# Henweiz/MARL-Responsible-Nav

Hardware: AMD Instinct MI355X
Metric: agent-env-steps/sec at 64k envs × 4 agents, 1/2/4/8 MI355X; HBM BW fraction (higher is better)
Workload: dtype int32

## Files before the change

### include/gridenv.h

```cpp
#ifndef GRIDENV_H
#define GRIDENV_H
#include <stdint.h>

#ifdef __cplusplus
extern "C" {
#endif

#define GW_MAX_AGENTS 8
#define GW_N_ACTIONS 9

typedef enum gw_status {
    GW_OK = 0,
    GW_ERR_ARG = -1,
    GW_ERR_HIP = -2,
    GW_ERR_ALLOC = -3,
    GW_ERR_STATE = -4
} gw_status;

typedef struct gw_scenario {
    int32_t H, W;
    const uint8_t *region;
    const uint8_t *policy_id;
    int32_t n_policies;
    const double *policy_cdf;
// ... 33 lines not shown
    int32_t *mdr;
    int32_t *final_pos;
    uint8_t *crash_bits;
    uint8_t *restr_bits;
    double *stats;
    uint8_t *done_copy;
    double *stats_acc;
    int64_t *tick;
    uint32_t *desc_copy;
    double *fear_row;
} gw_step_out;

#define GW_STATS 8

typedef struct gw_state {
    int32_t *pos;
    uint32_t *flags;
    int32_t *t;
    uint32_t *episode;
    int32_t *prev_dist;
    double *score;
    double *fear_score;
} gw_state;

gw_status gw_create(const gw_scenario *sc, const gw_config *cfg, int device, void **out_env);

gw_status gw_reset(void *env, const uint8_t *env_mask, const int32_t *spawn_cells, float *obs,
                   uint16_t *mask, void *stream);

gw_status gw_step(void *env, const int32_t *rl_actions, const int32_t *scripted,
                  const int32_t *spawn, const gw_step_out *out, void *stream);

gw_status gw_state_view(void *env, gw_state *out);

gw_status gw_copy_state(void *env, const gw_state *buf, int to_env, void *stream);

enum {
    GW_SPAN_STEP = 0, GW_SPAN_OBS = 1, GW_SPAN_FEAR = 2, GW_SPAN_ACT = 3, GW_SPAN_CNN_L1 = 4,
    GW_SPAN_CNN_LIST = 5, GW_SPAN_CNN_RARE = 6, GW_SPAN_WINDOW = 7, GW_SPAN_LEARN = 8,
    GW_SPAN_FEAR_ALT = 9, GW_SPAN_FEAL = 10, GW_SPAN_FEAR_FULL = 11, GW_SPAN_FEAR_PREVIEW = 12
};
gw_status gw_profile(void *env, int enable);
gw_status gw_profile_read(void *env, double out_ms[3], int64_t *n_steps);
gw_status gw_profile_spans(void *env, double *out, int64_t cap, int64_t *n_spans);

gw_status gw_fear_matrix(void *env, int64_t n, const int32_t *cells, const int32_t *actions,
                         const int32_t *mdr, const uint8_t *in_list, double *resp, int32_t *vm,
                         int32_t *va, double *feal, int32_t *feal_vm, int32_t *feal_va, void *stream);

int64_t gw_stats_rows(void *env);

int64_t gw_kernel_path(void *env);

gw_status gw_graph_replayed(void *env, void *stream);

int64_t gw_pipeline_state_bytes(void);
gw_status gw_pipeline_save(void *env, void *buf);
gw_status gw_pipeline_load(void *env, const void *buf, void *stream);

typedef struct gw_obs_source {
    const uint32_t *desc;
    const float *base;
    int32_t apples[GW_MAX_AGENTS];
    int32_t N, K, H, W, variant;
    int64_t E, env_offset;
} gw_obs_source;
gw_status gw_obs_view(void *env, gw_obs_source *out);

gw_status gw_obs_desc_copy(void *env, uint32_t *dst, void *stream);

gw_status gw_count_sims(void *env, uint64_t *counter);

gw_status gw_set_fear_alt(void *env, double *fear_alt);

gw_status gw_set_feal(void *env, double *feal, uint16_t *feal_valid);

gw_status gw_set_fear_full(void *env, double *resp_full, uint16_t *resp_valid);

gw_status gw_fear_preview(void *env, const int32_t *rl_actions, const int32_t *scripted, double *fear_alt,
                          int32_t *actions, int32_t *mdr, void *stream);

gw_status gw_obs_patch(void *env, int32_t P, float *patch, float *final_patch, void *stream);
gw_status gw_step_patch_next(void *env, int32_t P, float *patch, float *final_patch);

gw_status gw_set_obs_async(void *env, int enable);

enum { GW_OBS_F32 = 0, GW_OBS_BF16 = 1 };
gw_status gw_set_obs_dtype(void *env, int dtype);

#define GW_OBS_DESTS 8
gw_status gw_set_obs_delta(void *env, int on);
gw_status gw_obs_dest_forget(void *env, const void *ptr);
gw_status gw_obs_delta_counts(void *env, int64_t out[2]);

gw_status gw_set_fear_blocks(void *env, int wide);
gw_status gw_obs_fence(void *env, void *stream);
gw_status gw_fear_fence(void *env, void *stream);
void gw_set_last_error(const char *msg);
gw_status gw_dims(void *env, int64_t out[5]);

const char *gw_last_error(void);

void gw_destroy(void *env);

#ifdef __cplusplus
}
// ... 3 lines not shown
```

### marl-responsible-nav_amd/csrc/gridenv.hip

```cpp
#include <hip/hip_runtime.h>
#include <hip/hip_ext.h>

#include <cstdint>
#include <cstdio>
#include <cstdlib>
#include <algorithm>
#include <cstring>
#include <new>
#include <type_traits>
#include <string>
#include <vector>

#include "patch_ops.h"
#include "gridenv.h"
#include "prof.h"
#include "dispatch.h"
#include "obs_value.h"
#include "obs_dest.h"
#include "philox.h"
#include "window_rows.h"
#include "fear_alt_tasks.h"
#include "resp_tables.h"
#include "cf_env.h"

// ... 693 lines not shown
        nf = nw[1].x;
        ocells = ds[0];
        of = saved[e * NDESC + 4];
    }
    __syncthreads();
    if (!live || !(nf & D_WRITE)) return;
    if (k == 0) {
        uint4 *ds = reinterpret_cast<uint4 *>(saved + e * NDESC);
        ds[0] = nw[0];
        ds[1] = nw[1];
        ds[2] = nw[2];
    }
    PatchSet nu, od;
    decode_patches(p, nw[0], nf, k, nu);
    decode_patches(p, ocells, of, k, od);
    float *o = obs + ((int64_t)k * p.E + e) * HW;
#pragma unroll
    for (int q = 0; q < NPATCH_MAX; ++q) {
        const int c = nu.c[q];
        bool st = (unsigned)c < (unsigned)HW;
#pragma unroll
        for (int q2 = q + 1; q2 < NPATCH_MAX; ++q2) st = st && nu.c[q2] != c;
        bool held = false;
        float ov = 0.0f;
#pragma unroll
        for (int q2 = 0; q2 < NPATCH_MAX; ++q2) {
            const bool m = od.c[q2] == c;
            held = held || m;
            ov = m ? od.v[q2] : ov;
        }
        if (st && !(held && ov == nu.v[q])) o[c] = nu.v[q];
    }
#pragma unroll
    for (int q = 0; q < NPATCH_MAX; ++q) {
        const int c = od.c[q];
        bool st = (unsigned)c < (unsigned)HW;
#pragma unroll
        for (int q2 = 0; q2 < q; ++q2) st = st && od.c[q2] != c;
#pragma unroll
        for (int q2 = 0; q2 < NPATCH_MAX; ++q2) st = st && nu.c[q2] != c;
        if (st) o[c] = ((p.tb.roadbits[c >> 5] >> (c & 31)) & 1u) ? 0.0f : -1.0f;
    }
}

#ifndef GW_NOFEAR_BE
#define GW_NOFEAR_BE 32
#endif
#ifndef GW_DEF_BE
#define GW_DEF_BE 128
#endif
#ifndef GW_FEAR_T
#define GW_FEAR_T 256
#endif
template <int N, int KMAX, bool FEAR, bool WIDE = false, bool DEF = false, int TT = 128> struct V2Cfg {
    static constexpr int THREADS = TT;
    static constexpr int BE = (WIDE ? 2 : 1) *
        (FEAR ? (KMAX <= 2 ? (N <= 4 ? 32 : 16) : (N <= 4 ? 16 : 4))
              : (KMAX <= 2 && N > 4 ? 128 : (DEF && KMAX <= 2 ? GW_DEF_BE : GW_NOFEAR_BE)));
    static constexpr bool XDRAW = !FEAR && BE <= 32 && N <= 4;
    static_assert(!FEAR || BE * KMAX <= THREADS, "fear_block: one lane per (env, actor)");
    static_assert(!FEAR || BE <= 64, "task encoding holds 6 env bits");
    static constexpr int MAXB = FEAR ? BE * (1 + 2 * KMAX) : 1;
    static constexpr int MAXG = FEAR ? BE * KMAX * (N > 1 ? N - 1 : 1) : 1;
    using Task = typename std::conditional<(KMAX <= 2), uint16_t, uint32_t>::type;
    static __device__ __forceinline__ Task enc(int el, int k, int j, int var, int b) {
        return (Task)((uint32_t)el | ((uint32_t)b << 6) | ((uint32_t)var << 10) | ((uint32_t)j << 11) |
                      ((uint32_t)k << 14));
    }
};

template <int N, int KMAX, bool FEAR, bool WIDE = false, bool DEF = false, int TT = 128>
struct alignas(16) V2Shared {
    using Cfg = V2Cfg<N, KMAX, FEAR, WIDE, DEF, TT>;
    static constexpr int BE = Cfg::BE, FB = FEAR ? BE : 1;
    double red[Cfg::THREADS / 64][GW_STATS];
    typename Cfg::Task tasks[Cfg::MAXB];
    typename Cfg::Task groups[Cfg::MAXG];
    int pos[FB][N];
    int fin[FB][N];
    int apple[FB][KMAX];
    uint32_t bits[FB];
    int8_t act[FB][N];
    int8_t mdr[FB][N];
    uint8_t close[FB][KMAX];
    uint32_t vset[FB][KMAX][FEAR ? N : 1];
    uint2 wl[(N >= GW_LIST_MIN_N) ? Cfg::THREADS * N : 1];
    int8_t xact[Cfg::XDRAW ? BE : 1][N];
    int8_t xmdr[Cfg::XDRAW ? BE : 1][N];
    int nbase, ngroup;
};

#include "draw_action.h"

template <int N>
__device__ __forceinline__ void select_actions_v2(const Params &p, int64_t e, const EnvState<N> &es,
                                                  const uint32_t *ctab, const double *cdf_s, int (&act)[N]) {
#pragma unroll
    for (int n = 0; n < N; ++n) act[n] = draw_action(p, e, n, es.episode, es.t, es.pos[n], ctab, cdf_s);
}

template <int N, int KMAX, class Sh>
__device__ __forceinline__ void fear_plan_actor(const Params &p, Sh &sh, int el, int k, const int (&pos)[N],
                                                const int (&act)[N], int mdr_k, int off0) {
    using Cfg = typename Sh::Cfg;
    int pk = pos[0], ak = act[0];
#pragma unroll
    for (int n = 1; n < N; ++n) {
        pk = (n == k) ? pos[n] : pk;
        ak = (n == k) ? act[n] : ak;
    }
    uint32_t close = 0;
#pragma unroll
    for (int n = 0; n < N; ++n)
        if (n == k || manhattan(p, pk, pos[n]) <= 5) close |= 1u << n;
    sh.close[el][k] = (uint8_t)close;
#pragma unroll
    for (int n = 0; n < N; ++n) sh.vset[el][k][n] = 0u;
    if (ak == mdr_k) return;
    const int ng = __popc(close) - 1;
    int sb = off0 + atomicAdd(&sh.nbase, 2);
    int sg = ng ? atomicAdd(&sh.ngroup, ng) : 0;
    sh.tasks[sb] = Cfg::enc(el, k, 0, 0, 15);
    sh.tasks[sb + 1] = Cfg::enc(el, k, 0, 1, 15);
#pragma unroll
    for (int j = 0; j < N; ++j)
        if (j != k && ((close >> j) & 1u)) sh.groups[sg++] = Cfg::enc(el, k, j, 0, 0);
}

template <class Sh>
__device__ __forceinline__ uint32_t fear_task_at(const Sh &sh, int ti, int nb_end) {
    if (ti < nb_end) return sh.tasks[ti];
    const int g = (ti - nb_end) >> 4, s = (ti - nb_end) & 15;
    const uint32_t tk = sh.groups[g];
    const int el = tk & 63, j = (tk >> 11) & 7;
    const int bi = s & 7;
    const int b = bi + (bi >= (int)sh.act[el][j]);
    return tk | ((uint32_t)b << 6) | ((uint32_t)(s >> 3) << 10);
}

template <int N, class Sh>
__device__ __forceinline__ void fear_record(Sh &sh, int el, int k, int j, int var, int b, uint32_t valid) {
    const int sft = 16 * var;
    if (b != 15) {
        if ((valid >> j) & 1u) atomicOr(&sh.vset[el][k][j], 1u << (sft + b));
        return;
    }
    const uint32_t cl = sh.close[el][k];
#pragma unroll
    for (int n = 0; n < N; ++n) {
        if (n == k || !((valid >> n) & 1u)) continue;
        const uint32_t bits = ((cl >> n) & 1u) ? 1u << (int)sh.act[el][n] : 0x1FFu;
        atomicOr(&sh.vset[el][k][n], bits << sft);
    }
}

template <int N, int KMAX, class Sh, class OK>
__device__ __forceinline__ void fear_task(const Params &p, Sh &sh, uint32_t tk, const OK &okv) {
    const int el = tk & 63, b = (tk >> 6) & 15, var = (tk >> 10) & 1, j = (tk >> 11) & 7, k = (int)(tk >> 14);
    int pos[N], joint[N], fin[N];
    const uint32_t cl = sh.close[el][k];
#pragma unroll
    for (int n = 0; n < N; ++n) {
        pos[n] = sh.pos[el][n];
        joint[n] = ((cl >> n) & 1u) ? (int)sh.act[el][n] : 0;
        if (n == k && var == 0) joint[n] = sh.mdr[el][n];
        if (n == j && b != 15) joint[n] = b;
    }
    int apple[MAXN];
#pragma unroll
    for (int q = 0; q < MAXN; ++q) apple[q] = -1;
    constexpr bool LIST = N >= GW_LIST_MIN_N;
    World<N, LIST> w;
    w.init(pos, joint, p.W, p.w_magic);
    if constexpr (LIST) w.lw = &sh.wl[threadIdx.x * N];
    uint32_t caught;
    simulate<N, true>(w, okv, 0, apple, caught, fin);
    fear_record<N>(sh, el, k, j, var, b, ~(w.crash | w.restr) & ((1u << N) - 1u));
}

template <int N, int KMAX, class Sh>
__device__ __forceinline__ double fear_value(const Params &p, const Sh &sh, int el, int64_t e, int k, bool skipped,
                                             const double *resp_s) {
    double *row = p.out.fear_row ? p.out.fear_row + (e * p.K + k) * N : nullptr;
    if (skipped) {
        if (row)
#pragma unroll
            for (int jj = 0; jj < N; ++jj) row[jj] = 0.0;
        return 0.0;
    }
    double resp[N];
#pragma unroll
    for (int jj = 0; jj < N; ++jj) {
        resp[jj] = 0.0;
        if (jj != k) {
            const uint32_t v = sh.vset[el][k][jj];
            resp[jj] = resp_s[__popc(v & 0x1FFu) * 10 + __popc(v >> 16)];
        }
        if (row) row[jj] = resp[jj];
    }
    double sum = 0.0;
#pragma unroll
    for (int kk = 0; kk < KMAX; ++kk)
        if (kk == k) sum = np_sum_row<N>(resp, kk);
    return sum;
}

template <int T, uint32_t FM = 0xFFu, uint32_t IM = 0u>
__device__ __forceinline__ void block_stats(const Params &p, Contrib &ct, double (&red)[T / 64][GW_STATS], int tid,
                                            int64_t row) {
    const bool want = p.out.stats || p.out.stats_acc;
    if (want) {
        wave_sum_sel<FM, IM>(ct);
        if ((tid & 63) == 0)
#pragma unroll
            for (int i = 0; i < GW_STATS; ++i) red[tid >> 6][i] = ct.v[i];
    }
    __syncthreads();
    if (want && tid < GW_STATS) {
        double acc = red[0][tid];
#pragma unroll
        for (int w = 1; w < T / 64; ++w) acc = __dadd_rn(acc, red[w][tid]);
        stats_put(p.out, row * GW_STATS + tid, acc);
    }
}

#ifdef GW_STEP_CLK
__device__ unsigned long long g_step_clk[64][16];
#define STEP_STAMP(slot)                                                             \
    do {                                                                             \
        if (tid == 0 && bid < 64) g_step_clk[bid][slot] = clock64();                 \
    } while (0)
#else
#define STEP_STAMP(slot) \
    do {                 \
    } while (0)
#endif

template <int N, int KMAX, bool FEAR, bool DEFER>
__device__ __forceinline__ void step_v2_block(const Params &p, int64_t bid, V2Shared<N, KMAX, FEAR, false, DEFER> &sh,
                                              uint8_t *dyn) {
    using Cfg = V2Cfg<N, KMAX, FEAR, false, DEFER>;
    constexpr int BE = Cfg::BE, T = Cfg::THREADS;
    const double *cdf_s = p.lds_cdf ? reinterpret_cast<const double *>(dyn) : nullptr;
    uint32_t *ctab = reinterpret_cast<uint32_t *>(dyn + p.ctab_off);
    double *resp_s = reinterpret_cast<double *>(dyn + p.resp_off);
    const uint8_t *okb = nullptr;
    (void)okb;

    const int tid = threadIdx.x;
    if (p.e_begin + bid * BE >= p.e_end) return;
    const int64_t e0 = p.e_begin + bid * BE;
    const int nenv = (int)min((int64_t)BE, p.e_end - e0);
    const int K = p.K;
    STEP_STAMP(0);
#ifdef GW_STEP_CLK
    if (tid == 0 && bid < 64) g_step_clk[bid][15] = wall_clock64();
#endif
    if (e0 == 0 && tid == 0) step_tick(p.out);
    Contrib ct;
    contrib_zero(ct);
    EnvState<N> es;
    constexpr bool XDRAW = Cfg::XDRAW;
    constexpr int CPW = XDRAW ? BE / (T / 64) : 64;
    const int cel = XDRAW ? (((tid & 63) < CPW) ? (tid >> 6) * CPW + (tid & 63) : BE) : tid;
    if (cel < nenv) load_env<N>(p, e0 + cel, es);
    constexpr int NPAIR = XDRAW ? (BE * N + T - 1) / T : 1;
    int xpos[NPAIR], xt[NPAIR];
    uint32_t xep[NPAIR];
    if constexpr (XDRAW) {
#pragma unroll
        for (int j = 0; j < NPAIR; ++j) {
            const int i = tid + j * T, el = i % BE, n = i / BE;
            xpos[j] = xt[j] = 0;
            xep[j] = 0;
            if (n < N && el < nenv) {
                const int64_t e = e0 + el;
                xpos[j] = p.st.pos[(int64_t)n * p.E + e];
                xep[j] = p.st.episode[e];
                xt[j] = p.st.t[e];
            }
        }
    }
    lds_fill<T>(ctab, p.tb.celltab, p.HW, tid);
    if (p.lds_cdf)
        lds_fill<T>(reinterpret_cast<uint32_t *>(dyn), reinterpret_cast<const uint32_t *>(p.tb.cdf), 2 * p.n_cdf, tid);
    if (FEAR) lds_fill<T>(reinterpret_cast<uint32_t *>(resp_s), reinterpret_cast<const uint32_t *>(p.tb.resp), 200, tid);
    if (tid == 0) sh.nbase = sh.ngroup = 0;
    __syncthreads();
    STEP_STAMP(1);
// ... 124 lines not shown
            for (int k = 0; k < MAXN; ++k) apple[k] = (k < K && ((es.flags >> k) & 1u)) ? p.apples[k] : -1;
            constexpr bool LIST = N >= GW_LIST_MIN_N;
            World<N, LIST> w;
            w.init(pos, act, p.W, p.w_magic);
            if constexpr (LIST) w.lw = &sh.wl[tid * N];
            uint32_t caught;
            simulate<N, true>(w, okv, K, apple, caught, fin);
#ifdef GW_STEP_CLK
            if (bid < 64 && tid == 0) g_step_clk[bid][3] = clock64() + (uint64_t)(fin[0] + (int)caught < -1000);
#endif
            double fear[MAXN];
#pragma unroll
            for (int k = 0; k < MAXN; ++k) fear[k] = 0.0;
            ObsInfo<N> oi;
            finish_env<N, DEFER>(p, e, es, act, mdr, fear, w.crash, w.restr, fin, caught, ct, oi, ctab);
            if (!DEFER && p.out.fear_row) {
                double *row = p.out.fear_row + e * K * N;
                for (int i = 0; i < K * N; ++i) row[i] = 0.0;
            }
            STEP_STAMP(4);
            store_desc<N>(p, e, oi);
        }
    }

    constexpr uint32_t FM = DEFER ? 0u : ((1u << 0) | (1u << 5) | (FEAR ? (1u << 2) : 0u));
    STEP_STAMP(5);
    block_stats<T, FM, ST_INT>(p, ct, sh.red, tid, p.stats_row0 + e0 / BE);
    STEP_STAMP(6);
}

template <int N, int KMAX, bool FEAR, bool DEFER = false>
__global__ void __launch_bounds__(128) step_v2(Params p) {
    __shared__ V2Shared<N, KMAX, FEAR, false, DEFER> sh;
    extern __shared__ __attribute__((aligned(16))) uint8_t dyn[];
    step_v2_block<N, KMAX, FEAR, DEFER>(p, blockIdx.x, sh, dyn);
}


template <int N, int KMAX, bool FEAR>
__global__ void __launch_bounds__(128) step_obs(Params p, Params q, float *__restrict__ obs,
                                                float *__restrict__ final_obs, uint32_t nstep) {
    __shared__ V2Shared<N, KMAX, FEAR> sh;
    extern __shared__ __attribute__((aligned(16))) uint8_t dyn[];
    const bool is_step = blockIdx.x < nstep;
    const uint32_t rb = is_step ? blockIdx.x : blockIdx.x - nstep;
    if (is_step)
        step_v2_block<N, KMAX, FEAR, false>(p, rb, sh, dyn);
    else if (q.obs_bf16)
        obs_block<128, true, true, true>(q, obs, final_obs, rb, reinterpret_cast<uint32_t *>(dyn));
    else
        obs_block<128, true, true, false>(q, obs, final_obs, rb, reinterpret_cast<uint32_t *>(dyn));
}

template <int N, int KMAX, bool WIDE, int T>
__device__ __forceinline__ void fear_block(const Params &p, uint32_t bid) {
    using Cfg = V2Cfg<N, KMAX, true, WIDE, false, T>;
    using Sh = V2Shared<N, KMAX, true, WIDE, false, T>;
    constexpr int BE = Cfg::BE;
    __shared__ Sh sh;
    __shared__ double xfear[KMAX][BE];
    extern __shared__ __attribute__((aligned(16))) uint8_t dyn[];
    uint32_t *ctab = reinterpret_cast<uint32_t *>(dyn + p.ctab_off);
    double *resp_s = reinterpret_cast<double *>(dyn + p.resp_off);

    const int tid = threadIdx.x;
    if (p.e_begin + (int64_t)bid * BE >= p.e_end) return;
    const int64_t e0 = p.e_begin + (int64_t)bid * BE;
    const int nenv = (int)min((int64_t)BE, p.e_end - e0);
    const int K = p.K;
    STEP_STAMP(8);
    const int el = tid % BE, ka = tid / BE;
    const bool live = ka < KMAX && ka < K && el < nenv, tail = tid < nenv;
    int pos[N], act[N], rew[MAXN];
    uint32_t bonus = 0;
    bool done = false;
    double score0 = 0.0, fscore0 = 0.0;
    if (live) load_fear_rec<N>(p, e0 + el, pos, act, rew, bonus, done);
    if (tail) {
        score0 = p.st.score[e0 + tid];
        fscore0 = p.st.fscore[e0 + tid];
    }
    lds_fill<T>(ctab, p.tb.celltab, p.HW, tid);
    lds_fill<T>(reinterpret_cast<uint32_t *>(resp_s), reinterpret_cast<const uint32_t *>(p.tb.resp), 200, tid);
    if (tid == 0) sh.nbase = sh.ngroup = 0;
    __syncthreads();
    STEP_STAMP(9);
    const CtabOk okv{ctab};
    bool skipped = true;
    if (live) {
        int mdr_k = 0;
#pragma unroll
        for (int n = 0; n < N; ++n) {
            const int m = (int)((ctab[pos[n]] >> CT_MDR) & 0xFu);
            if (n == ka) {
                mdr_k = m;
                skipped = act[n] == m;
            }
            if (tail) {
                sh.pos[el][n] = pos[n];
                sh.act[el][n] = (int8_t)act[n];
                sh.mdr[el][n] = (int8_t)m;
            }
        }
        fear_plan_actor<N, KMAX>(p, sh, el, ka, pos, act, mdr_k, 0);
    }
    __syncthreads();
    STEP_STAMP(10);
    const int nb_end = sh.nbase, ntask = nb_end + 16 * sh.ngroup;
    if (tid == 0 && p.sims && ntask) atomicAdd(p.sims, (unsigned long long)ntask);
    for (int ti = tid; ti < ntask; ti += T) fear_task<N, KMAX>(p, sh, fear_task_at(sh, ti, nb_end), okv);
    __syncthreads();
    STEP_STAMP(11);
    if (live) xfear[ka][el] = fear_value<N, KMAX>(p, sh, el, e0 + el, ka, skipped, resp_s);
    __syncthreads();
    Contrib ct;
    contrib_zero(ct);
    if (tail) {
        const int64_t e = e0 + tid;
        double shaped[MAXN], fsum_in[MAXN];
#pragma unroll
        for (int k = 0; k < MAXN; ++k) {
            shaped[k] = fsum_in[k] = 0.0;
            if (k >= K || k >= KMAX) continue;
            const double fear = xfear[k][tid];
            const double r = ((bonus >> k) & 1u) ? __dadd_rn((double)rew[k], 0.1) : (double)rew[k];
            shaped[k] = __dadd_rn(__dmul_rn(p.fear_weight, fear), r);
            fsum_in[k] = fear;
        }
        const double score = __dadd_rn(score0, np_sum_small(shaped, K));
        const double fscore = __dadd_rn(fscore0, np_sum_small(fsum_in, K));
        const gw_step_out &o = p.out;
#pragma unroll
        for (int k = 0; k < KMAX; ++k) {
            if (k >= K) continue;
            const int64_t ek = e * K + k;
            if (o.fear) o.fear[ek] = fsum_in[k];
            if (o.shaped) o.shaped[ek] = shaped[k];
        }
        if (o.ep_return) o.ep_return[e] = score;
        if (o.ep_fear) o.ep_fear[e] = fscore;
        const bool fresh = done && p.auto_reset;
        p.st.score[e] = fresh ? 0.0 : score;
        p.st.fscore[e] = fresh ? 0.0 : fscore;
        ct.v[0] = done ? score : 0.0;
        ct.v[2] = np_sum_small(fsum_in, K);
        ct.v[5] = np_sum_small(shaped, K);
    }
    STEP_STAMP(12);
    block_stats<T, ST_F64_FEAR, 0u>(p, ct, sh.red, tid, p.stats_row0 + e0 / BE);
    STEP_STAMP(13);
}

template <int N, int KMAX, bool WIDE>
__global__ void __launch_bounds__(WIDE ? GW_FEAR_T : 128) fear_v2(Params p) {
    fear_block<N, KMAX, WIDE, WIDE ? GW_FEAR_T : 128>(p, blockIdx.x);
}

template <int N, int KMAX, bool WIDE>
__global__ void __launch_bounds__(128) fear_rows_kernel(Params p, PatchArgs a, uint32_t nfear, uint32_t nrx) {
    if (blockIdx.x < nfear) {
        fear_block<N, KMAX, WIDE, 128>(p, blockIdx.x);
        return;
    }
    extern __shared__ __attribute__((aligned(16))) uint8_t dynr[];
    const uint32_t r = blockIdx.x - nfear;
    gwrows::rows_block<N + 1, 16, 2, 2>(a, r % nrx, (int)(r / nrx), reinterpret_cast<float4 (*)[64 * 4]>(dynr));
}

template <int N>
__global__ void __launch_bounds__(CF_T) fear_alt_kernel(Params p, double *__restrict__ table) {
    constexpr bool LIST = N >= GW_LIST_MIN_N;
    constexpr int VBW = fear_alt::bit_words(N, N);
    static_assert(fear_alt::max_per_env(4, 2) == 450 && fear_alt::max_per_env(8, 2) == 1026, "task maxima");
    static_assert(VBW == N * NA * N && VBW <= 576, "valid-bit sets: [K <= N][9][N] words per env");
    static_assert(fear_alt::max_per_env(N, N) <= 4104, "tasks per env fit an int with room");
    __shared__ uint32_t vb[CF_WAVES][VBW];
    __shared__ uint2 wl[LIST ? CF_T * N : 1];
    __shared__ unsigned int s_nsim;
    static_assert(sizeof(uint32_t) * CF_WAVES * VBW + sizeof(uint2) * (LIST ? CF_T * N : 1) <= 26 * 1024,
                  "static LDS of fear_alt_kernel");
    CfEnv<N> c;
    c.begin(p, 0, s_nsim, [&] { for (int i = c.lane; i < VBW; i += 64) vb[c.wave][i] = 0u; });
    const int (&pos)[N] = c.pos, (&act)[N] = c.act, (&mdr)[N] = c.mdr;
    const int tid = threadIdx.x, wave = c.wave, lane = c.lane, K = min(p.K, N);
    const CtabOk okv{c.ctab};
    uint32_t close[N];
    int tcount[N], ntask = 0;
#pragma unroll
    for (int k = 0; k < N; ++k) {
        close[k] = 0u;
        tcount[k] = 0;
        if (k >= K) continue;
#pragma unroll
        for (int n = 0; n < N; ++n)
            if (n == k || manhattan(p, pos[k], pos[n]) <= 5) close[k] |= 1u << n;
        tcount[k] = fear_alt::per_actor(__popc(close[k]));
        ntask += tcount[k];
    }
    if (!c.live) ntask = 0;

    for (int ti = lane; ti < ntask; ti += 64) {
        int k = 0, r = ti;
#pragma unroll
        for (int q = 0; q < N - 1; ++q)
            if (q == k && q < K - 1 && r >= tcount[q]) {
                r -= tcount[q];
                ++k;
            }
// ... 174 lines not shown
    if (tid < N) {
        const int m = __popc(s_bits[N + N * (N - 1) + tid]), a = __popc(s_bits[tid]);
        if (q.feal) q.feal[e * N + tid] = q.tab[100 + m * 10 + a];
        if (q.feal_vm) q.feal_vm[e * N + tid] = m;
        if (q.feal_va) q.feal_va[e * N + tid] = a;
    }
}

}

namespace {

thread_local std::string g_err;

gw_status fail(gw_status s, const std::string &msg) {
    g_err = msg;
    return s;
}

#define HIP_TRY(expr)                                                                      \
    do {                                                                                   \
        hipError_t _e = (expr);                                                            \
        if (_e != hipSuccess) return fail(GW_ERR_HIP, std::string(#expr) + ": " + hipGetErrorString(_e)); \
    } while (0)

#define GW_TRY(expr)                   \
    do {                               \
        gw_status _s = (expr);         \
        if (_s != GW_OK) return _s;    \
    } while (0)

enum KernelPath : int {
    PATH_DEFER = 3,
    PATH_MERGED = 4,
};

struct Env {
    int device = 0;
    int H = 0, W = 0, HW = 0, N = 0, K = 0, F = 0, P = 0;
    int64_t E = 0, env_offset = 0;
    int fear = 0, max_steps = 0, auto_reset = 1, variant = 0;
    double fear_weight = 0.0;
    uint64_t seed = 0;
    int apples[GW_MAX_AGENTS] = {0};
    bool initialized = false;
    KernelPath mode = PATH_DEFER;
    int obs_be = 2;
    bool obs_bf16 = false;
    int obs_be_f32 = 2;
    uint32_t *celltab = nullptr;
    uint32_t *roadbits = nullptr;
    bool fear_wide = true;
    bool fear_wide_fixed = false;
    hipStream_t aux = nullptr;
    std::vector<hipEvent_t> sync_ev;
    bool obs_async = false;
    hipStream_t last_stream = nullptr;
    bool obs_lazy = false;
    int obs_chunks = 1;
    struct PatchReq {
        bool armed = false, done = false;
        int P = 0;
        float *patch = nullptr, *final_patch = nullptr;
    } patch_req;
    hipStream_t obs_stream = nullptr;
    hipStream_t obs_stream2 = nullptr;
    int obs_streams = 2;
    int obs_cur = 0;
    const void *obs_last[2] = {nullptr, nullptr};
    hipEvent_t obs_done[2] = {nullptr, nullptr};
    bool obs_pending[2] = {false, false};
    hipEvent_t world_ev = nullptr;
    bool fear_async = false;
    bool fear_pending = false;
    hipEvent_t fear_ev = nullptr;
    bool obs_queued = false;
    bool qobs_prof = false;
    int qobs_buf = 0;
    gw::Params qobs;
    uint32_t *desc_buf[2] = {nullptr, nullptr};
    int dcur = 0;
    bool obs_delta = false;
    gwdest::Table dests;
    uint32_t *dest_desc[gwdest::SLOTS] = {nullptr};
    hipEvent_t dest_ev[gwdest::SLOTS] = {nullptr};
    hipStream_t dest_stream[gwdest::SLOTS] = {nullptr};
    bool dest_written[gwdest::SLOTS] = {false};
    int64_t n_obs_full = 0, n_obs_delta = 0;
    uint8_t *okmask = nullptr, *policy = nullptr, *mdr = nullptr;
    double *cdf = nullptr, *resp = nullptr;
    uint16_t *amask = nullptr;
    int32_t *free_cells = nullptr;
    float *base = nullptr;
    int32_t *pos = nullptr, *t = nullptr, *prev = nullptr;
    uint32_t *flags = nullptr, *episode = nullptr, *desc = nullptr;
    uint4 *fwork = nullptr;
    unsigned long long *sims = nullptr;
    double *fear_alt = nullptr;
    double *feal = nullptr;
    uint16_t *feal_valid = nullptr;
    double *resp_full = nullptr;
    uint16_t *resp_valid = nullptr;
    uint4 *preview_rec = nullptr;
    std::vector<std::pair<int, float *>> ptbls;
    double *score = nullptr, *fscore = nullptr;
    std::vector<void *> allocs;
// ... 180 lines not shown
    }
    for (int k = 0; k < GW_MAX_AGENTS; ++k) p.apples[k] = env->apples[k];
    return p;
}

template <typename R, typename F>
R with_variant(const Env *env, R bad, F &&f) {
    return gw::with_agents(env->N, bad, [&](auto n) {
        using Two = std::integral_constant<int, 2>;
        if (env->fear_wide) return env->K <= 2 ? f(n, Two{}, std::true_type{}) : f(n, n, std::true_type{});
        return env->K <= 2 ? f(n, Two{}, std::false_type{}) : f(n, n, std::false_type{});
    });
}

struct BlockEnvs { int step, fear; };

BlockEnvs block_envs(const Env *env) {
    return with_variant(env, BlockEnvs{0, 0}, [&](auto n, auto kmax, auto wide) {
        constexpr int N = decltype(n)::value, KMAX = decltype(kmax)::value;
        if (defer_fear(env))
            return BlockEnvs{gw::V2Cfg<N, KMAX, false, false, true>::BE,
                             gw::V2Cfg<N, KMAX, true, decltype(wide)::value>::BE};
        return BlockEnvs{env->fear ? gw::V2Cfg<N, KMAX, true>::BE : gw::V2Cfg<N, KMAX, false>::BE, 0};
    });
}

int64_t ceil_div(int64_t n, int64_t d) { return (n + d - 1) / d; }

size_t step_lds(const gw::Params &p, bool fear) { return (size_t)p.resp_off + (fear ? 100 * sizeof(double) : 0); }

size_t fear_lds(gw::Params &p) {
    p.lds_cdf = 0;
    p.ctab_off = 0;
    p.resp_off = celltab_lds(p.HW);
    return (size_t)p.resp_off + 100 * sizeof(double);
}

hipError_t launch_step(const Env *env, const gw::Params &p, hipStream_t s) {
    const int64_t count = p.e_end - p.e_begin;
    if (count <= 0) return hipSuccess;
    return with_variant(env, hipErrorInvalidValue, [&](auto n, auto kmax, auto) {
        constexpr int N = decltype(n)::value, KMAX = decltype(kmax)::value;
        const dim3 grid((unsigned)ceil_div(count, block_envs(env).step)), block(gw::V2Cfg<N, KMAX, false>::THREADS);
        if (defer_fear(env))
            gw_launch((gw::step_v2<N, KMAX, false, true>), grid, block, step_lds(p, false), s, p);
        else if (env->fear)
            gw_launch((gw::step_v2<N, KMAX, true>), grid, block, step_lds(p, true), s, p);
        else
            gw_launch((gw::step_v2<N, KMAX, false>), grid, block, step_lds(p, false), s, p);
        return hipGetLastError();
    });
}

hipError_t launch_fear(const Env *env, const gw::Params &p0, hipStream_t s, const gw::PatchArgs *a = nullptr) {
    gw::Params p = p0;
    const size_t dyn = fear_lds(p);
    const int64_t count = p.e_end - p.e_begin;
    if (!a && count <= 0) return hipSuccess;
    return with_variant(env, hipErrorInvalidValue, [&](auto n, auto kmax, auto wide) {
        constexpr int N = decltype(n)::value, KMAX = decltype(kmax)::value;
        constexpr bool WIDE = decltype(wide)::value;
        const BlockEnvs be = block_envs(env);
        p.stats_row0 = ceil_div(env->E, be.step);
        const unsigned nfear = (unsigned)ceil_div(count, be.fear);
        if (a) {
            const unsigned nrx = (unsigned)((a->E * a->P + 255) / 256);
            gw_launch((gw::fear_rows_kernel<N, KMAX, WIDE>), dim3(nfear + nrx * (unsigned)a->K), dim3(128),
                      std::max(dyn, sizeof(float4) * 2 * 64 * 4), s, p, *a, nfear, nrx);
        } else {
            gw_launch((gw::fear_v2<N, KMAX, WIDE>), dim3(nfear), dim3(WIDE ? GW_FEAR_T : 128), dyn,
                      s, p);
        }
        return hipGetLastError();
    });
}

template <typename F>
gw_status launch_cf(Env *env, int kind, const gw::Params &p0, F &&launch) {
    gw::Params p = p0;
    const size_t dyn = fear_lds(p);
    const int64_t count = p.e_end - p.e_begin;
    SpanGuard span(env, env->profiling, kind);
    GW_TRY(span.status);
    if (count <= 0) return GW_OK;
    const hipError_t launched = gw::with_agents(env->N, hipErrorInvalidValue, [&](auto n) {
        launch(n, dim3((unsigned)ceil_div(count, gw::CF_WAVES)), dim3(gw::CF_T), dyn, p);
        return hipGetLastError();
    });
    HIP_TRY(launched);
    return GW_OK;
}

hipError_t launch_reset(const Env *env, const gw::Params &p, hipStream_t s) {
    return gw::with_agents(env->N, hipErrorInvalidValue, [&](auto n) {
        gw_launch((gw::reset_kernel<decltype(n)::value>), dim3((unsigned)ceil_div(env->E, 256)), dim3(256), 0, s, p);
        return hipGetLastError();
    });
}

hipError_t launch_fear_matrix(const Env *env, int64_t n_blocks, const gw::FmParams &q, hipStream_t s) {
    return gw::with_agents(env->N, hipErrorInvalidValue, [&](auto n) -> hipError_t {
        constexpr int N = decltype(n)::value;
        if constexpr (N >= 2) {
            gw_launch((gw::fear_matrix_kernel<N>), dim3((unsigned)n_blocks), dim3(128), (size_t)celltab_lds(env->HW), s, q);
            return hipGetLastError();
        } else {
            return hipErrorInvalidValue;
        }
    });
}

size_t obs_lds_bytes(const Env *env) {
    const size_t base = sizeof(uint32_t) * ((env->HW + 31) / 32 + gw::OBS_BE) +
                        (size_t)2 * 2 * env->obs_be * env->K * (env->N + 1) * sizeof(uint32_t);
    if (env->obs_bf16 || !gw::obs_tab_ok(env->HW, env->obs_be, env->K)) return base;
    return (size_t)gw::obs_ent_off(env->HW, env->obs_be, env->K, env->N + 1) +
           (size_t)env->obs_be * env->K * (env->N + 1) * sizeof(float4) +
           (size_t)gw::obs_tab_bytes(env->HW, env->obs_be, env->K);
}

hipError_t launch_step_obs(const Env *env, const gw::Params &p, const gw::Params &q, hipStream_t s) {
// ... 421 lines not shown
        if (!road(r, q + 1)) m &= ~(1u << 4);
        if (!road(r - 2, q)) m &= ~(1u << 5);
        if (!road(r + 2, q)) m &= ~(1u << 6);
        if (!road(r, q - 2)) m &= ~(1u << 7);
        if (!road(r, q + 2)) m &= ~(1u << 8);
        am[c] = m;
        base[c] = sc->region[c] ? 0.0f : -1.0f;
        if (sc->region[c]) freec.push_back(c);
        if (sc->mdr[c] >= GW_N_ACTIONS) return fail(GW_ERR_ARG, "MdR action out of range");
        if (sc->policy_id[c] >= sc->n_policies) return fail(GW_ERR_ARG, "policy id out of range");
        mdr[c] = sc->mdr[c];
        pol[c] = sc->policy_id[c];
        ctab[c] = (uint32_t)pol[c] | ((uint32_t)mdr[c] << 8) | ((uint32_t)m << 12) | ((uint32_t)(ok[c] & 0xFu) << 21) |
                  ((uint32_t)(sc->region[c] != 0) << 25);
        if (sc->region[c]) rbits[c >> 5] |= 1u << (c & 31);
    }
    if ((int)freec.size() < N) return fail(GW_ERR_ARG, "fewer road cells than agents");
    for (int k = 0; k < K; ++k)
        if (sc->apples[k] < 0 || sc->apples[k] >= HW) return fail(GW_ERR_ARG, "apple outside the grid");
    double resp_tab[200];
    gwtab::fill(resp_tab);
    if (!gwtab::resp_diag_zero(resp_tab)) return fail(GW_ERR_STATE, "Resp table: a diagonal entry is not 0.0");
    const std::vector<double> resp(resp_tab, resp_tab + 200);

    Env *env = new (std::nothrow) Env();
    if (!env) return fail(GW_ERR_ALLOC, "host allocation failed");
    env->device = device;
    env->H = H; env->W = W; env->HW = HW; env->N = N; env->K = K;
    env->F = (int)freec.size();
    env->P = sc->n_policies;
    env->E = cfg->num_envs;
    env->env_offset = cfg->env_offset;
    env->fear = cfg->fear ? 1 : 0;
    env->fear_weight = cfg->fear_weight;
    env->max_steps = cfg->max_steps;
    env->auto_reset = cfg->auto_reset ? 1 : 0;
    env->variant = cfg->variant;
    env->seed = cfg->seed;
    for (int k = 0; k < K; ++k) env->apples[k] = sc->apples[k];
    {
        const char *kv = std::getenv("GW_KERNEL");
        env->mode = PATH_DEFER;
        if (HW % 4 == 0) {
            const char *mb = std::getenv("GW_MERGE_BYTES");
            const int64_t lim = mb ? std::atoll(mb) : ((int64_t)160 << 20);
            if (cfg->num_envs * (int64_t)K * HW * 4 <= lim) env->mode = PATH_MERGED;
            if (kv && std::strcmp(kv, "merged") == 0) env->mode = PATH_MERGED;
        }
        if (kv && std::strcmp(kv, "defer") == 0) env->mode = PATH_DEFER;
        const char *fb = std::getenv("GW_FEAR_BE");
        if (fb && std::strcmp(fb, "wide") == 0) env->fear_wide = true;
        if (fb && std::strcmp(fb, "narrow") == 0) env->fear_wide = false;
        env->fear_wide_fixed = fb != nullptr;
        int be_def = std::max(1, 4096 / std::max(1, K * HW));
        if (defer_fear(env)) be_def *= 2;
        env->obs_be = std::max(1, std::min(8, be_def));
        env->obs_be_f32 = env->obs_be;
        const char *oc = std::getenv("GW_OBS_CHUNKS");
        if (oc) env->obs_chunks = std::max(1, std::min(64, std::atoi(oc)));
        const char *osn = std::getenv("GW_OBS_STREAMS");
        if (osn) env->obs_streams = std::atoi(osn) > 1 ? 2 : 1;
    }

    auto cleanup = [&](gw_status s) {
        for (void *p : env->allocs) (void)hipFree(p);
        delete env;
        return s;
    };
    if (hipSetDevice(device) != hipSuccess) return cleanup(fail(GW_ERR_HIP, "hipSetDevice failed"));
    const size_t E = (size_t)env->E;
    gw_status st = GW_OK;
    if ((st = dalloc(env, &env->okmask, HW)) || (st = dalloc(env, &env->policy, HW)) ||
        (st = dalloc(env, &env->mdr, HW)) || (st = dalloc(env, &env->cdf, (size_t)env->P * 2 * 9)) ||
        (st = dalloc(env, &env->resp, 200)) || (st = dalloc(env, &env->amask, HW)) ||
        (st = dalloc(env, &env->free_cells, freec.size())) || (st = dalloc(env, &env->base, HW)) ||
        (st = dalloc(env, &env->pos, (size_t)N * E)) || (st = dalloc(env, &env->t, E)) ||
        (st = dalloc(env, &env->prev, (size_t)K * E)) || (st = dalloc(env, &env->flags, E)) ||
        (st = dalloc(env, &env->episode, E)) || (st = dalloc(env, &env->desc, 2 * E * gw::NDESC)) ||
        (st = dalloc(env, &env->score, E)) || (st = dalloc(env, &env->fscore, E)) ||
        (st = dalloc(env, &env->celltab, HW)) || (st = dalloc(env, &env->roadbits, rbits.size())) ||
        (defer_fear(env) && (st = dalloc(env, &env->fwork, E * (N <= 4 ? 1 : 2)))))
        return cleanup(st);
    hipError_t he = hipSuccess;
#define CP(dst, src, n) if (he == hipSuccess) he = hipMemcpy(dst, src, n, hipMemcpyHostToDevice)
    CP(env->okmask, ok.data(), HW);
    CP(env->policy, pol.data(), HW);
    CP(env->mdr, mdr.data(), HW);
    CP(env->cdf, sc->policy_cdf, sizeof(double) * env->P * 2 * 9);
    CP(env->resp, resp.data(), sizeof(double) * 200);
    CP(env->amask, am.data(), sizeof(uint16_t) * HW);
    CP(env->free_cells, freec.data(), sizeof(int32_t) * freec.size());
    CP(env->base, base.data(), sizeof(float) * HW);
    CP(env->celltab, ctab.data(), sizeof(uint32_t) * HW);
    CP(env->roadbits, rbits.data(), sizeof(uint32_t) * rbits.size());
#undef CP
    if (he == hipSuccess) he = hipMemset(env->episode, 0xFF, sizeof(uint32_t) * E);
    if (he == hipSuccess) he = hipMemset(env->desc, 0, sizeof(uint32_t) * 2 * E * gw::NDESC);
    env->desc_buf[0] = env->desc;
    env->desc_buf[1] = env->desc + E * gw::NDESC;
    if (he == hipSuccess) he = hipDeviceSynchronize();
    if (he != hipSuccess) return cleanup(fail(GW_ERR_HIP, std::string("init: ") + hipGetErrorString(he)));
    *out_env = env;
    return GW_OK;
}

gw_status gw_reset(void *handle, const uint8_t *env_mask, const int32_t *spawn_cells, float *obs,
                   uint16_t *mask, void *stream) {
    Env *env = static_cast<Env *>(handle);
    if (!env) return fail(GW_ERR_ARG, "null env");
    env->patch_req = Env::PatchReq{};
    gw::Params p = make_params(env);
    p.rmask = env_mask;
    p.spawn = spawn_cells;
    p.out.mask = mask;
    hipStream_t s = static_cast<hipStream_t>(stream);
    GW_TRY(wait_obs(env, s));
    env->dests.forget(nullptr);
    HIP_TRY(launch_reset(env, p, s));
    HIP_TRY(launch_obs(env, p, obs, nullptr, s));
    env->initialized = true;
    return GW_OK;
}
// ... 45 lines not shown
    GW_TRY(wait_obs(env, static_cast<hipStream_t>(stream)));
    return GW_OK;
}

gw_status gw_set_obs_dtype(void *handle, int dtype) {
    Env *env = static_cast<Env *>(handle);
    if (!env) return fail(GW_ERR_ARG, "null env");
    if (dtype != GW_OBS_F32 && dtype != GW_OBS_BF16) return fail(GW_ERR_ARG, "gw_set_obs_dtype: unknown dtype");
    if (dtype == GW_OBS_BF16 && env->HW % 8 != 0)
        return fail(GW_ERR_ARG, "gw_set_obs_dtype: bf16 obs needs H*W % 8 == 0");
    const bool bf = dtype == GW_OBS_BF16;
    if (bf != env->obs_bf16) GW_TRY(drain_writers(env));
    env->dests.forget(nullptr);
    env->obs_be = bf ? std::max(1, std::min(gw::OBS_BE, 32768 / std::max(1, env->K * env->HW)))
                 : env->obs_be_f32;
    env->obs_bf16 = bf;
    if (!env->initialized && !env->fear_wide_fixed) env->fear_wide = !bf;
    return GW_OK;
}

gw_status gw_set_fear_blocks(void *handle, int wide) {
    Env *env = static_cast<Env *>(handle);
    if (!env) return fail(GW_ERR_ARG, "null env");
    if (env->initialized) return fail(GW_ERR_STATE, "gw_set_fear_blocks after gw_reset (the stats rows follow it)");
    if (!env->fear_wide_fixed) env->fear_wide = wide != 0;
    return GW_OK;
}

gw_status gw_fear_fence(void *handle, void *stream) {
    Env *env = static_cast<Env *>(handle);
    if (!env) return fail(GW_ERR_ARG, "null env");
    GW_TRY(wait_fear(env, static_cast<hipStream_t>(stream)));
    return GW_OK;
}

gw_status gw_profile(void *handle, int enable) {
    Env *env = static_cast<Env *>(handle);
    if (!env) return fail(GW_ERR_ARG, "null env");
    env->profiling = enable != 0;
    const size_t want = env->profiling ? env->ev_used + (size_t)std::max(enable, 32) : 0;
    while (env->ev_pool.size() < want) {
        hipEvent_t e = nullptr;
        HIP_TRY(hipEventCreateWithFlags(&e, env->prof_flags));
        env->ev_pool.push_back(e);
    }
    return GW_OK;
}

#ifdef GW_STEP_CLK
int gw_step_debug_clocks(unsigned long long *out) {
    return hipMemcpyFromSymbol(out, HIP_SYMBOL(gw::g_step_clk), sizeof(unsigned long long) * 64 * 16) == hipSuccess
               ? 0 : -1;
}
#endif

gw_status gw_profile_spans(void *handle, double *out, int64_t cap, int64_t *n_spans) {
    Env *env = static_cast<Env *>(handle);
    if (!env || !n_spans || (cap > 0 && !out)) return fail(GW_ERR_ARG, "null argument");
    *n_spans = (int64_t)env->spans.size();
    if (env->spans.empty() || cap <= 0) return GW_OK;
    const hipEvent_t t0 = env->ev_pool[env->spans.front().b];
    for (size_t i = 0; i < env->spans.size() && (int64_t)i < cap; ++i) {
        const Env::Span &sp = env->spans[i];
        HIP_TRY(hipEventSynchronize(env->ev_pool[sp.e]));
        float b = 0.f, e = 0.f;
        HIP_TRY(hipEventElapsedTime(&b, t0, env->ev_pool[sp.b]));
        HIP_TRY(hipEventElapsedTime(&e, t0, env->ev_pool[sp.e]));
        out[3 * i + 0] = (double)sp.kind;
        out[3 * i + 1] = (double)b;
        out[3 * i + 2] = (double)e;
    }
    return GW_OK;
}

gw_status gw_profile_read(void *handle, double out_ms[3], int64_t *n_steps) {
    Env *env = static_cast<Env *>(handle);
    if (!env || !out_ms) return fail(GW_ERR_ARG, "null argument");
    out_ms[0] = out_ms[1] = out_ms[2] = 0.0;
    for (const Env::Span &sp : env->spans) {
        HIP_TRY(hipEventSynchronize(env->ev_pool[sp.e]));
        float ms = 0.f;
        HIP_TRY(hipEventElapsedTime(&ms, env->ev_pool[sp.b], env->ev_pool[sp.e]));
        if (sp.kind >= 0 && sp.kind < 3) out_ms[sp.kind] += ms;
    }
    if (n_steps) *n_steps = env->steps_timed;
    env->spans.clear();
    env->ev_used = 0;
    env->steps_timed = 0;
    return GW_OK;
}

gw_status gw_state_view(void *handle, gw_state *out) {
    Env *env = static_cast<Env *>(handle);
    if (!env || !out) return fail(GW_ERR_ARG, "null argument");
    out->pos = env->pos;
    out->flags = env->flags;
    out->t = env->t;
    out->episode = env->episode;
    out->prev_dist = env->prev;
    out->score = env->score;
    out->fear_score = env->fscore;
    return GW_OK;
}

gw_status gw_copy_state(void *handle, const gw_state *buf, int to_env, void *stream) {
    Env *env = static_cast<Env *>(handle);
// ... 193 lines not shown
    st.mode = env->mode;
    st.desc = env->desc;
    std::memcpy(buf, &st, sizeof(st));
    return GW_OK;
}

gw_status gw_pipeline_load(void *handle, const void *buf, void *stream) {
    Env *env = static_cast<Env *>(handle);
    if (!env || !buf) return fail(GW_ERR_ARG, "null argument");
    PipeState st;
    std::memcpy(&st, buf, sizeof(st));
    if (st.mode != env->mode) return fail(GW_ERR_ARG, "gw_pipeline_load: state of another kernel path");
    if (env->mode != PATH_MERGED && (env->obs_async || st.obs_queued))
        return fail(GW_ERR_STATE, "gw_pipeline_load: only the merged path's async pipeline (or synchronous obs)");
    env->dests.forget(nullptr);
    env->qobs = st.qobs;
    env->qobs_buf = st.qobs_buf;
    env->dcur = st.dcur;
    env->desc = st.desc;
    env->obs_queued = st.obs_queued != 0;
    env->qobs_prof = false;
    env->last_stream = static_cast<hipStream_t>(stream);
    return GW_OK;
}

gw_status gw_set_obs_delta(void *handle, int on) {
    Env *env = static_cast<Env *>(handle);
    if (!env) return fail(GW_ERR_ARG, "null env");
    env->dests.forget(nullptr);
    env->obs_delta = on != 0;
    return GW_OK;
}

gw_status gw_obs_dest_forget(void *handle, const void *ptr) {
    Env *env = static_cast<Env *>(handle);
    if (!env) return fail(GW_ERR_ARG, "null env");
    env->dests.forget(ptr);
    return GW_OK;
}

gw_status gw_obs_delta_counts(void *handle, int64_t out[2]) {
    Env *env = static_cast<Env *>(handle);
    if (!env || !out) return fail(GW_ERR_ARG, "null argument");
    out[0] = env->n_obs_full;
    out[1] = env->n_obs_delta;
    return GW_OK;
}

int64_t gw_kernel_path(void *handle) {
    const Env *env = static_cast<const Env *>(handle);
    return env ? env->mode : -1;
}

gw_status gw_dims(void *handle, int64_t out[5]) {
    Env *env = static_cast<Env *>(handle);
    if (!env || !out) return fail(GW_ERR_ARG, "null argument");
    out[0] = env->H; out[1] = env->W; out[2] = env->N; out[3] = env->K; out[4] = env->E;
    return GW_OK;
}

void gw_destroy(void *handle) {
    Env *env = static_cast<Env *>(handle);
    if (!env) return;
    (void)hipSetDevice(env->device);
    (void)hipDeviceSynchronize();
    for (hipEvent_t e : env->ev_pool) (void)hipEventDestroy(e);
    for (hipEvent_t e : env->sync_ev) (void)hipEventDestroy(e);
    if (env->aux) (void)hipStreamDestroy(env->aux);
    if (env->obs_stream) (void)hipStreamDestroy(env->obs_stream);
    if (env->obs_stream2) (void)hipStreamDestroy(env->obs_stream2);
    for (hipEvent_t e : env->obs_done)
        if (e) (void)hipEventDestroy(e);
    if (env->world_ev) (void)hipEventDestroy(env->world_ev);
    if (env->fear_ev) (void)hipEventDestroy(env->fear_ev);
    for (hipEvent_t e : env->dest_ev)
        if (e) (void)hipEventDestroy(e);
    for (void *p : env->allocs) (void)hipFree(p);
    delete env;
}

}
```

Measured before the change: 5.290 billion.

## Pool four wide FeAR blocks into one 1024-thread workgroup for large grids

Adds a pooled FeAR kernel in which one workgroup covers PL times as many envs (PL defaults to 4, 1024 threads), widening the task encoding to 8 env bits and using 32-bit tasks. Stats are reduced per 64-env group so the per-row stats layout stays the same. The pooled kernel is chosen automatically when the env count fills every CU several times over, or forced through the env setting. The aim is to balance uneven per-env FeAR task counts across a larger block and to cut block scheduling overhead. In exchange it uses more LDS per block, has coarser occupancy, and adds debug timestamp hooks.

```diff
diff --git a/include/gridenv.h b/include/gridenv.h
--- a/include/gridenv.h
+++ b/include/gridenv.h
@@ -109,6 +109,8 @@
 
 int64_t gw_kernel_path(void *env);
 
+int gw_fear_pooled(void *env);
+
 gw_status gw_graph_replayed(void *env, void *stream);
 
 int64_t gw_pipeline_state_bytes(void);
diff --git a/marl-responsible-nav_amd/csrc/gridenv.hip b/marl-responsible-nav_amd/csrc/gridenv.hip
--- a/marl-responsible-nav_amd/csrc/gridenv.hip
+++ b/marl-responsible-nav_amd/csrc/gridenv.hip
@@ -769,26 +769,31 @@
 #ifndef GW_FEAR_T
 #define GW_FEAR_T 256
 #endif
-template <int N, int KMAX, bool FEAR, bool WIDE = false, bool DEF = false, int TT = 128> struct V2Cfg {
+#ifndef GW_FEAR_POOL
+#define GW_FEAR_POOL 4
+#endif
+template <int N, int KMAX, bool FEAR, bool WIDE = false, bool DEF = false, int TT = 128, int PL = 1> struct V2Cfg {
     static constexpr int THREADS = TT;
-    static constexpr int BE = (WIDE ? 2 : 1) *
+    static constexpr int BE = PL * (WIDE ? 2 : 1) *
         (FEAR ? (KMAX <= 2 ? (N <= 4 ? 32 : 16) : (N <= 4 ? 16 : 4))
               : (KMAX <= 2 && N > 4 ? 128 : (DEF && KMAX <= 2 ? GW_DEF_BE : GW_NOFEAR_BE)));
     static constexpr bool XDRAW = !FEAR && BE <= 32 && N <= 4;
     static_assert(!FEAR || BE * KMAX <= THREADS, "fear_block: one lane per (env, actor)");
-    static_assert(!FEAR || BE <= 64, "task encoding holds 6 env bits");
+    static constexpr int EB = BE <= 64 ? 6 : 8;
+    static_assert(!FEAR || BE <= (1 << EB), "task encoding holds EB env bits");
+    static_assert(PL == 1 || (FEAR && WIDE), "only the wide FeAR blocks are pooled");
     static constexpr int MAXB = FEAR ? BE * (1 + 2 * KMAX) : 1;
     static constexpr int MAXG = FEAR ? BE * KMAX * (N > 1 ? N - 1 : 1) : 1;
-    using Task = typename std::conditional<(KMAX <= 2), uint16_t, uint32_t>::type;
+    using Task = typename std::conditional<(KMAX <= 2 && EB == 6), uint16_t, uint32_t>::type;
     static __device__ __forceinline__ Task enc(int el, int k, int j, int var, int b) {
-        return (Task)((uint32_t)el | ((uint32_t)b << 6) | ((uint32_t)var << 10) | ((uint32_t)j << 11) |
-                      ((uint32_t)k << 14));
+        return (Task)((uint32_t)el | ((uint32_t)b << EB) | ((uint32_t)var << (EB + 4)) | ((uint32_t)j << (EB + 5)) |
+                      ((uint32_t)k << (EB + 8)));
     }
 };
 
-template <int N, int KMAX, bool FEAR, bool WIDE = false, bool DEF = false, int TT = 128>
+template <int N, int KMAX, bool FEAR, bool WIDE = false, bool DEF = false, int TT = 128, int PL = 1>
 struct alignas(16) V2Shared {
-    using Cfg = V2Cfg<N, KMAX, FEAR, WIDE, DEF, TT>;
+    using Cfg = V2Cfg<N, KMAX, FEAR, WIDE, DEF, TT, PL>;
     static constexpr int BE = Cfg::BE, FB = FEAR ? BE : 1;
     double red[Cfg::THREADS / 64][GW_STATS];
     typename Cfg::Task tasks[Cfg::MAXB];
@@ -847,12 +852,13 @@
 template <class Sh>
 __device__ __forceinline__ uint32_t fear_task_at(const Sh &sh, int ti, int nb_end) {
     if (ti < nb_end) return sh.tasks[ti];
+    constexpr int EB = Sh::Cfg::EB;
     const int g = (ti - nb_end) >> 4, s = (ti - nb_end) & 15;
     const uint32_t tk = sh.groups[g];
-    const int el = tk & 63, j = (tk >> 11) & 7;
+    const int el = tk & ((1 << EB) - 1), j = (tk >> (EB + 5)) & 7;
     const int bi = s & 7;
     const int b = bi + (bi >= (int)sh.act[el][j]);
-    return tk | ((uint32_t)b << 6) | ((uint32_t)(s >> 3) << 10);
+    return tk | ((uint32_t)b << EB) | ((uint32_t)(s >> 3) << (EB + 4));
 }
 
 template <int N, class Sh>
@@ -873,7 +879,9 @@
 
 template <int N, int KMAX, class Sh, class OK>
 __device__ __forceinline__ void fear_task(const Params &p, Sh &sh, uint32_t tk, const OK &okv) {
-    const int el = tk & 63, b = (tk >> 6) & 15, var = (tk >> 10) & 1, j = (tk >> 11) & 7, k = (int)(tk >> 14);
+    constexpr int EB = Sh::Cfg::EB;
+    const int el = tk & ((1 << EB) - 1), b = (tk >> EB) & 15, var = (tk >> (EB + 4)) & 1, j = (tk >> (EB + 5)) & 7,
+              k = (int)(tk >> (EB + 8));
     int pos[N], joint[N], fin[N];
     const uint32_t cl = sh.close[el][k];
 #pragma unroll
@@ -947,11 +955,40 @@
     do {                                                                             \
         if (tid == 0 && bid < 64) g_step_clk[bid][slot] = clock64();                 \
     } while (0)
+constexpr int FEAR_GRID_MAX = 4096;
+__device__ unsigned long long g_fear_grid[FEAR_GRID_MAX][4];
+#define FEAR_GRID_STAMP(slot, value)                                                 \
+    do {                                                                             \
+        if (tid == 0 && bid < FEAR_GRID_MAX) g_fear_grid[bid][slot] = (value);       \
+    } while (0)
 #else
 #define STEP_STAMP(slot) \
     do {                 \
     } while (0)
+#define FEAR_GRID_STAMP(slot, value) \
+    do {                             \
+    } while (0)
 #endif
+
+template <int G, uint32_t FM, uint32_t IM>
+__device__ __forceinline__ void pooled_stats(const Params &p, Contrib &ct, double (*red)[GW_STATS], int tid, int64_t row0,
+                                             int ngroup) {
+    const bool want = p.out.stats || p.out.stats_acc;
+    if (want && tid < 64 * G) {
+        wave_sum_sel<FM, IM>(ct);
+        if ((tid & 63) == 0)
+#pragma unroll
+            for (int i = 0; i < GW_STATS; ++i) red[tid >> 6][i] = ct.v[i];
+    }
+    __syncthreads();
+    if (want && tid < G * GW_STATS && tid / GW_STATS < ngroup) {
+        const int g = tid / GW_STATS, i = tid % GW_STATS;
+        double acc = red[g][i];
+#pragma unroll
+        for (int w = 1; w < GW_FEAR_T / 64; ++w) acc = __dadd_rn(acc, 0.0);
+        stats_put(p.out, (row0 + g) * GW_STATS + i, acc);
+    }
+}
 
 template <int N, int KMAX, bool FEAR, bool DEFER>
 __device__ __forceinline__ void step_v2_block(const Params &p, int64_t bid, V2Shared<N, KMAX, FEAR, false, DEFER> &sh,
@@ -1182,13 +1219,14 @@
         obs_block<128, true, true, false>(q, obs, final_obs, rb, reinterpret_cast<uint32_t *>(dyn));
 }
 
-template <int N, int KMAX, bool WIDE, int T>
+template <int N, int KMAX, bool WIDE, int T, int PL = 1>
 __device__ __forceinline__ void fear_block(const Params &p, uint32_t bid) {
-    using Cfg = V2Cfg<N, KMAX, true, WIDE, false, T>;
-    using Sh = V2Shared<N, KMAX, true, WIDE, false, T>;
+    using Cfg = V2Cfg<N, KMAX, true, WIDE, false, T, PL>;
+    using Sh = V2Shared<N, KMAX, true, WIDE, false, T, PL>;
     constexpr int BE = Cfg::BE;
     __shared__ Sh sh;
     __shared__ double xfear[KMAX][BE];
+    static_assert(sizeof(Sh) + sizeof(double) * KMAX * BE <= 48 * 1024, "fear_block: static LDS");
     extern __shared__ __attribute__((aligned(16))) uint8_t dyn[];
     uint32_t *ctab = reinterpret_cast<uint32_t *>(dyn + p.ctab_off);
     double *resp_s = reinterpret_cast<double *>(dyn + p.resp_off);
@@ -1199,6 +1237,7 @@
     const int nenv = (int)min((int64_t)BE, p.e_end - e0);
     const int K = p.K;
     STEP_STAMP(8);
+    FEAR_GRID_STAMP(0, wall_clock64());
     const int el = tid % BE, ka = tid / BE;
     const bool live = ka < KMAX && ka < K && el < nenv, tail = tid < nenv;
     int pos[N], act[N], rew[MAXN];
@@ -1238,6 +1277,7 @@
     STEP_STAMP(10);
     const int nb_end = sh.nbase, ntask = nb_end + 16 * sh.ngroup;
     if (tid == 0 && p.sims && ntask) atomicAdd(p.sims, (unsigned long long)ntask);
+    FEAR_GRID_STAMP(2, (unsigned long long)ntask);
     for (int ti = tid; ti < ntask; ti += T) fear_task<N, KMAX>(p, sh, fear_task_at(sh, ti, nb_end), okv);
     __syncthreads();
     STEP_STAMP(11);
@@ -1277,13 +1317,26 @@
         ct.v[5] = np_sum_small(shaped, K);
     }
     STEP_STAMP(12);
-    block_stats<T, ST_F64_FEAR, 0u>(p, ct, sh.red, tid, p.stats_row0 + e0 / BE);
+    if constexpr (PL == 1)
+        block_stats<T, ST_F64_FEAR, 0u>(p, ct, sh.red, tid, p.stats_row0 + e0 / BE);
+    else
+        pooled_stats<PL, ST_F64_FEAR, 0u>(p, ct, sh.red, tid, p.stats_row0 + e0 / (BE / PL), (nenv + 63) / 64);
     STEP_STAMP(13);
+    FEAR_GRID_STAMP(1, wall_clock64());
 }
 
 template <int N, int KMAX, bool WIDE>
 __global__ void __launch_bounds__(WIDE ? GW_FEAR_T : 128) fear_v2(Params p) {
     fear_block<N, KMAX, WIDE, WIDE ? GW_FEAR_T : 128>(p, blockIdx.x);
+}
+
+template <int N, int KMAX>
+constexpr bool FEAR_POOLABLE = GW_FEAR_POOL > 1 && GW_FEAR_T == 256 && GW_FEAR_T * GW_FEAR_POOL <= 1024 &&
+                               V2Cfg<N, KMAX, true, true>::BE == 64;
+
+template <int N, int KMAX>
+__global__ void __launch_bounds__(GW_FEAR_T * GW_FEAR_POOL) fear_v2_pool(Params p) {
+    fear_block<N, KMAX, true, GW_FEAR_T * GW_FEAR_POOL, GW_FEAR_POOL>(p, blockIdx.x);
 }
 
 template <int N, int KMAX, bool WIDE>
@@ -1564,6 +1617,8 @@
     uint32_t *roadbits = nullptr;
     bool fear_wide = true;
     bool fear_wide_fixed = false;
+    int fear_pool = -1;
+    int num_cus = 256;
     hipStream_t aux = nullptr;
     std::vector<hipEvent_t> sync_ev;
     bool obs_async = false;
@@ -1850,6 +1905,12 @@
     });
 }
 
+template <int N, int KMAX, bool WIDE>
+bool fear_pooled(const Env *env, int64_t count) {
+    if (!WIDE || !gw::FEAR_POOLABLE<N, KMAX> || env->fear_pool == 0) return false;
+    return env->fear_pool > 0 || count >= (int64_t)64 * GW_FEAR_POOL * env->num_cus;
+}
+
 hipError_t launch_fear(const Env *env, const gw::Params &p0, hipStream_t s, const gw::PatchArgs *a = nullptr) {
     gw::Params p = p0;
     const size_t dyn = fear_lds(p);
@@ -1865,6 +1926,10 @@
             const unsigned nrx = (unsigned)((a->E * a->P + 255) / 256);
             gw_launch((gw::fear_rows_kernel<N, KMAX, WIDE>), dim3(nfear + nrx * (unsigned)a->K), dim3(128),
                       std::max(dyn, sizeof(float4) * 2 * 64 * 4), s, p, *a, nfear, nrx);
+        } else if (fear_pooled<N, KMAX, WIDE>(env, count)) {
+            if constexpr (WIDE && gw::FEAR_POOLABLE<N, KMAX>)
+                gw_launch((gw::fear_v2_pool<N, KMAX>), dim3((unsigned)ceil_div(count, be.fear * GW_FEAR_POOL)),
+                          dim3(GW_FEAR_T * GW_FEAR_POOL), dyn, s, p);
         } else {
             gw_launch((gw::fear_v2<N, KMAX, WIDE>), dim3(nfear), dim3(WIDE ? GW_FEAR_T : 128), dyn,
                       s, p);
@@ -2392,6 +2457,10 @@
         if (fb && std::strcmp(fb, "wide") == 0) env->fear_wide = true;
         if (fb && std::strcmp(fb, "narrow") == 0) env->fear_wide = false;
         env->fear_wide_fixed = fb != nullptr;
+        if (fb && (std::strcmp(fb, "pool") == 0 || std::strcmp(fb, "wide64") == 0)) {
+            env->fear_wide = true;
+            env->fear_pool = std::strcmp(fb, "pool") == 0 ? 1 : 0;
+        }
         int be_def = std::max(1, 4096 / std::max(1, K * HW));
         if (defer_fear(env)) be_def *= 2;
         env->obs_be = std::max(1, std::min(8, be_def));
@@ -2408,6 +2477,8 @@
         return s;
     };
     if (hipSetDevice(device) != hipSuccess) return cleanup(fail(GW_ERR_HIP, "hipSetDevice failed"));
+    if (hipDeviceGetAttribute(&env->num_cus, hipDeviceAttributeMultiprocessorCount, device) != hipSuccess || env->num_cus <= 0)
+        return cleanup(fail(GW_ERR_HIP, "hipDeviceGetAttribute(multiprocessor count) failed"));
     const size_t E = (size_t)env->E;
     gw_status st = GW_OK;
     if ((st = dalloc(env, &env->okmask, HW)) || (st = dalloc(env, &env->policy, HW)) ||
@@ -2559,6 +2630,11 @@
     return hipMemcpyFromSymbol(out, HIP_SYMBOL(gw::g_step_clk), sizeof(unsigned long long) * 64 * 16) == hipSuccess
                ? 0 : -1;
 }
+int gw_fear_debug_grid(unsigned long long *out, int64_t nblocks) {
+    if (nblocks < 0 || nblocks > gw::FEAR_GRID_MAX) return -1;
+    return hipMemcpyFromSymbol(out, HIP_SYMBOL(gw::g_fear_grid), sizeof(unsigned long long) * 4 * (size_t)nblocks) == hipSuccess
+               ? 0 : -1;
+}
 #endif
 
 gw_status gw_profile_spans(void *handle, double *out, int64_t cap, int64_t *n_spans) {
@@ -2858,6 +2934,15 @@
     return env ? env->mode : -1;
 }
 
+int gw_fear_pooled(void *handle) {
+    const Env *env = static_cast<const Env *>(handle);
+    if (!env) return -1;
+    if (!defer_fear(env)) return 0;
+    return with_variant(env, 0, [&](auto n, auto kmax, auto wide) {
+        return (int)fear_pooled<decltype(n)::value, decltype(kmax)::value, decltype(wide)::value>(env, env->E);
+    });
+}
+
 gw_status gw_dims(void *handle, int64_t out[5]) {
     Env *env = static_cast<Env *>(handle);
     if (!env || !out) return fail(GW_ERR_ARG, "null argument");
```

Result: slower. 5.117 billion (-3.3%).
